# DiamondLightSource/fast-feedback-service

Hardware: AMD Instinct MI355X
Metric: detector frames/s (Eiger-16M 4362x4148 uint16) (higher is better)
Workload: dtype u16; 1 GPU; eiger16m: 4148x4362 uint16, 7x7 dispersion window, 32 frames/step/GPU resident in HBM, spots+centroids returned to host; streams=4, parallelism=single GPU, spot_gather=none (single GPU)

## Files before the change

fast-feedback-service_amd/csrc/ffs_context.hip:

```cpp
#include <sys/mman.h>

#include "ffs_internal.hpp"
#include "kernels_mask.hpp"

static_assert(sizeof(ReflOut) == sizeof(ffs_reflection), "record layout");
static_assert(offsetof(ReflOut, sum_intensity) == offsetof(ffs_reflection, sum_intensity), "record layout");

thread_local std::string g_create_error;

static void ctx_destroy_internal(ffs_ctx* c);
namespace {
struct Registry {
    std::mutex mu;
    std::unordered_set<const void*> live[3];
    std::atomic<bool> exiting{false};
    bool exit_hook_installed = false;
};
Registry& registry() {
    static Registry* r = new Registry();
    return *r;
}
static void on_process_exit() {
    Registry& r = registry();
    std::vector<ffs_ctx*> ctxs;
// ... 131 lines not shown
    }
    const uint64_t npx = (uint64_t)width * height;
    c->cap = max_strong ? max_strong : (uint32_t)std::min<uint64_t>(npx, 1u << 18);
    c->cap = (uint32_t)std::min<uint64_t>(c->cap, npx);
    c->max_comp = std::min<uint32_t>(c->cap, 1u << 14);
    c->n_tiles = ((int)height + kTileRows - 1) / kTileRows;
    ffs_default_params(&c->params);
    if (hipSetDevice(device) != hipSuccess) {
        g_create_error = "hipSetDevice failed";
        delete c;
        return FFS_ERR_DEVICE;
    }
    hipError_t e = hipMalloc(&c->d_maskbits, L.plane_frame_stride + 256);
    if (e == hipSuccess) e = hipMalloc(&c->d_ginfo, (size_t)(L.H + kInfoExtraRows) * ginfo_pitch(L, pixel_bytes) + 256);
    if (e == hipSuccess) e = hipMalloc(&c->d_mmap, (size_t)L.H * L.pitch_px + 256);
    if (e != hipSuccess) {
        g_create_error = std::string("hipMalloc(mask): ") + hipGetErrorString(e);
        ctx_destroy_internal(c);
        return FFS_ERR_NOMEM;
    }
    c->chain_ok = chain_prepare_device();
    {
        int lo = 0, hi = 0;
        hipError_t es = hipDeviceGetStreamPriorityRange(&lo, &hi);
        if (es == hipSuccess) es = hipStreamCreateWithPriority(&c->dense_st, hipStreamNonBlocking, (lo + hi) / 2);
        if (es == hipSuccess) es = hipStreamCreateWithFlags(&c->up_st, hipStreamNonBlocking);
        for (auto& sp : c->sparse_st)
            if (es == hipSuccess) es = hipStreamCreateWithPriority(&sp, hipStreamNonBlocking, hi);
        if (es == hipSuccess)
            for (auto& e : c->chain_ev)
// ... 97 lines not shown

static void ctx_destroy_internal(ffs_ctx* c) {
    (void)hipSetDevice(c->device);
    ahead_stop(c, true);
    for (auto* st : c->stack_pool) stack3d_free(st);
    c->stack_pool.clear();
    if (AssemblyPool* pool = c->assembly.exchange(nullptr)) {
        pool->owner.lock();
        pool->owner.unlock();
        delete pool;
    }
    if (c->d_maskbits) (void)hipFree(c->d_maskbits);
    if (c->d_gain_map) (void)hipFree(c->d_gain_map);
    if (c->d_ginfo) (void)hipFree(c->d_ginfo);
    if (c->d_mmap) (void)hipFree(c->d_mmap);
    if (c->dense_st) (void)hipStreamDestroy(c->dense_st);
    if (c->dense_st2) (void)hipStreamDestroy(c->dense_st2);
    if (c->d_handoff) (void)hipFree(c->d_handoff);
    if (c->up_st) (void)hipStreamDestroy(c->up_st);
    for (auto st : c->sparse_st) if (st) (void)hipStreamDestroy(st);
    for (auto e : c->chain_ev) if (e) (void)hipEventDestroy(e);
    for (auto& pb : c->pinned_pool) pinned_free(pb);
    delete c;
}

static int rebuild_mask_tables(ffs_ctx* c) {
    const Layout& L = c->L;
    const uint32_t gpitch = ginfo_pitch(L, c->pixel_bytes);
    HIP_TRY(c, hipMemset(c->d_ginfo, 0, (size_t)(L.H + kInfoExtraRows) * gpitch));
    const int groups = L.pitch_px / (c->pixel_bytes == 2 ? 8 : 4);
    (void)hipGetLastError();
    if (c->pixel_bytes == 2)
        hipLaunchKernelGGL(k_build_maps, dim3((groups + 255) / 256, L.H), dim3(256), 0, 0, c->d_maskbits, L.mpitch, L.W, L.H,
                           L.pitch_px, c->d_mmap, c->d_ginfo, gpitch);
    else
        hipLaunchKernelGGL(k_build_maps4, dim3((groups + 255) / 256, L.H), dim3(256), 0, 0, c->d_maskbits, L.mpitch, L.W, L.H,
                           L.pitch_px, c->d_mmap, c->d_ginfo, gpitch);
    HIP_TRY(c, hipGetLastError());
    HIP_TRY(c, hipDeviceSynchronize());
    return FFS_OK;
}

static int ffs_ctx_set_mask_impl(ffs_ctx* c, const uint8_t* host_mask) {
    if (!c) return FFS_ERR_INVALID;
    const Layout& L = c->L;
    std::vector<uint8_t> bits(L.plane_frame_stride, 0);
    const int full = L.W / 8;
    for (int y = 0; y < L.H; ++y) {
        uint8_t* row = bits.data() + (size_t)y * L.mpitch;
        if (host_mask) {
            const uint8_t* m = host_mask + (size_t)y * L.W;
            for (int g = 0; g < full; ++g) {
                uint64_t v;
                std::memcpy(&v, m + 8 * g, 8);
// ... 209 lines not shown
    else if (k == "sched") { if ((ok = (value == 0 || value == 3) && c->n_streams_made == 0)) t.sched = (int)value; }
    else if (k == "chain_first") { if ((ok = in(0, 64))) t.chain_first = (int)value; }
    else if (k == "bright_cap") { if ((ok = in(0, kBrightCap))) t.bright_cap = (int)value; }
    else if (k == "frames_per_group") { if ((ok = in(1, 1 << 30))) t.frames_per_group = (int)value; }
    else if (k == "target_waves") { if ((ok = in(1, 1 << 24))) t.target_waves = value; }
    else if (k == "stream_bands") { if ((ok = in(0, 4096))) t.stream_bands = (int)value; }
    else if (k == "dense_mask") { if ((ok = in(0, 1))) t.dense_mask = (int)value; }
    else if (k == "occupancy_bitmap") { if ((ok = in(0, 1))) t.occupancy_bitmap = (int)value; }
    else if (k == "direct_records") { if ((ok = in(0, 1) && c->n_streams_made == 0)) t.direct_records = (int)value; }
    else if (k == "decode_in_dense_stream") { if ((ok = in(0, 1))) t.decode_in_dense_stream = (int)value; }
    else if (k == "ext_fused") { if ((ok = in(0, 1))) t.ext_fused = (int)value; }
    else if (k == "ext_erode") { if ((ok = in(0, 2))) t.ext_erode = (int)value; }
    else if (k == "ext_e_sparse") { if ((ok = in(0, 1))) t.ext_e_sparse = (int)value; }
    else if (k == "ext_rest_aside") { if ((ok = in(0, 1))) t.ext_rest_aside = (int)value; }
    else if (k == "band_taper") { if ((ok = in(0, 99))) t.band_taper = (int)value; }
    else if (k == "rows_ahead") { if ((ok = in(2, 4))) t.rows_ahead = (int)value; }
    else if (k == "ccl_grid") { if ((ok = in(1, 1024))) t.ccl_grid = (int)value; }
    else {
        c->err = "ffs_ctx_set_tuning: unknown key '" + k + "'";
        return FFS_ERR_INVALID;
    }
    if (!ok) {
        c->err = "ffs_ctx_set_tuning: value out of range for '" + k + "' (sched / direct_records: before the first stream is created)";
        return FFS_ERR_INVALID;
    }
    return FFS_OK;
}


extern "C" void ffs_stream_destroy(ffs_stream* s) {
// ... 260 lines not shown
```

fast-feedback-service_amd/csrc/ffs_device.h:

```cpp
#pragma once
#include <hip/hip_runtime.h>
#include <stdint.h>

#include "launch_geometry.hpp"
#include "threshold_route.hpp"

#ifdef FFS_EXPERIMENTS
#define FFS_DBG(args, bit) (((args).dbg & (bit)) != 0)
#define FFS_STOP_AFTER(A, phase) if ((A).stop_after == (phase)) return
#define FFS_PHASE_TS(A, idx) do { if ((A).phase_ts && threadIdx.x == 0) (A).phase_ts[(size_t)blockIdx.x * 8 + (idx)] = wall_clock64(); } while (0)
#else
#define FFS_PHASE_TS(A, idx) do {} while (0)
#define FFS_DBG(args, bit) false
#define FFS_STOP_AFTER(A, phase) do {} while (0)
#endif

namespace ffsamd {

constexpr int kInfoExtraRows = 3;

constexpr int kWlogCap = 256;
constexpr int kTileRows = 8;
constexpr int kExactListCap = 2048;

// ... 21 lines not shown
    uint32_t ib2, is2;
    uint32_t thr_floor;
    int bright_to_plane;
    uint8_t* dplane;
    uint8_t* eplane;
    int eplane_clean;
    int ext_strips, ext_band_rows, ext_bands;
    int ext_flavour;
    int ext_variant;
    const uint8_t* ginfo;
    const uint8_t* mmap;
    uint32_t gpitch;
    int gpf;
    int n_frames;
    int group_frames;
    int s_strips, s_band_rows, s_bands;
    uint32_t* bright_n;
    uint2* bright_list;
    uint32_t bright_cap;
    uint32_t* overflow;
    uint32_t* occ;
    uint32_t occ_frame_words;
    uint32_t occ_spr;
    int dense_mask;
    uint2* wlog;
    uint32_t* wlog_n;
    uint4* wpix;
    uint32_t* handoff;
    uint32_t handoff_seq;
    int dbg_prio;
    int dbg;
// ... 157 lines not shown
```

fast-feedback-service_amd/csrc/ffs_internal.hpp:

```cpp
#pragma once
#include <algorithm>
#include <atomic>
#include <chrono>
#include <condition_variable>
#include <functional>
#include <cmath>
#include <cstdio>
#include <cstdlib>
#include <cstring>
#include <deque>
#include <map>
#include <mutex>
#include <new>
#include <string>
#include <thread>
#include <unordered_set>
#include <vector>

#include <hip/hip_runtime.h>
#include <hip/hip_ext.h>

#include "ffs_hip.h"
#include "ffs_device.h"
#include "threshold_route.hpp"
// ... 64 lines not shown
    Layout L{};
    int pixel_bytes = 2;
    uint32_t max_batch = 1;
    uint32_t cap = 0;
    uint32_t max_comp = 0;
    int n_tiles = 0;
    ffs_params params{};
    int max_valid_scope = FFS_MAX_VALID_CENTRE;
    double gain = 0.0;
    float* d_gain_map = nullptr;
    bool has_gain_map = false;
    float gain_map_min = 0.0f, gain_map_max = 0.0f;
    uint8_t* d_maskbits = nullptr;
    uint8_t* d_ginfo = nullptr;
    uint8_t* d_mmap = nullptr;
    hipStream_t dense_st = nullptr;
    hipStream_t dense_st2 = nullptr;
    uint32_t* d_handoff = nullptr;
    std::mutex dense_mu;
    uint32_t handoff_seq = 0;
    int handoff_last = -1;
    hipStream_t up_st = nullptr;
    hipStream_t sparse_st[2] = {nullptr, nullptr};
    int n_streams_made = 0;
    std::mutex stream_mu;
    std::vector<ffs_stream*> live_streams;
    std::vector<ffs_stack3d*> live_stacks;
    std::vector<ffs_stack3d*> stack_pool;
    std::vector<struct PinnedBuf> pinned_pool;
    std::atomic<int> inflight{0};
// ... 19 lines not shown
    ffs_stream* big = nullptr;
    std::vector<OverflowFrame> ovf;
    bool lists_valid = true;
    bool log_off = false;
    uint2* d_wlog = nullptr;
    uint32_t* d_wlog_n = nullptr;
    uint4* d_wpix = nullptr;
    size_t wlog_waves = 0;
    uint4* d_band_hdr = nullptr;
    uint8_t* d_band_acc = nullptr;
    uint32_t* d_band_seam = nullptr;
    uint32_t band_slots = 0;
    uint32_t band_backoff = 0;
    uint32_t path_bits = 0;
    uint32_t reruns = 0;
    bool runs_overflowed = false;
    uint32_t *d_pack_k = nullptr, *d_pack_i = nullptr;
    StackSlice *d_pack_tab = nullptr, *h_pack_tab = nullptr;
    hipEvent_t ev_pack = nullptr;
    hipEvent_t ev_sent = nullptr;
    int ev_sent_dev = -1;
    bool sent_pending = false;
    hipStream_t st = nullptr;
    hipStream_t st_up = nullptr;
    bool st2_shared = false;
    bool st_shared = false;
    hipStream_t st2 = nullptr;
    hipEvent_t ev[7] = {};
    uint8_t* d_slab = nullptr;
    uint8_t* d_img = nullptr;
// ... 174 lines not shown
```

fast-feedback-service_amd/csrc/ffs_submit.hip:

```cpp
#include "ffs_internal.hpp"
#include "kernels_threshold.hpp"
#include "kernels_extended.hpp"
#include "kernels_stream.hpp"
#include "kernels_ccl.hpp"
#include "kernels_chain.hpp"
#include "kernels_band.hpp"
#include "kernels_decode.hpp"
#include "kernels_byteoffset.hpp"
#include "kernels_window.hpp"

bool chain_prepare_device() {
    const hipError_t e1 = hipFuncSetAttribute(reinterpret_cast<const void*>(&k_frame_chain<uint16_t>), hipFuncAttributeMaxDynamicSharedMemorySize, kChainDynBytes);
    const hipError_t e2 = hipFuncSetAttribute(reinterpret_cast<const void*>(&k_frame_chain<uint32_t>), hipFuncAttributeMaxDynamicSharedMemorySize, kChainDynBytes);
    const hipError_t e3 = hipFuncSetAttribute(reinterpret_cast<const void*>(&k_frame_chain<uint16_t, true>), hipFuncAttributeMaxDynamicSharedMemorySize, kChainDynBytes);
    const hipError_t e4 = hipFuncSetAttribute(reinterpret_cast<const void*>(&k_frame_chain<uint16_t, false, true>), hipFuncAttributeMaxDynamicSharedMemorySize, kChainDynBytes);
    const hipError_t e5 = hipFuncSetAttribute(reinterpret_cast<const void*>(&k_frame_chain<uint32_t, false, true>), hipFuncAttributeMaxDynamicSharedMemorySize, kChainDynBytes);
    (void)hipGetLastError();
    return e1 == hipSuccess && e2 == hipSuccess && e3 == hipSuccess && e4 == hipSuccess && e5 == hipSuccess;
}

ThresholdRoute batch_route(const ffs_stream* s, const Rerun& how) {
    const ParamSnapshot& b = s->batch;
    return threshold_route(b.params.algorithm, s->ctx->pixel_bytes, win_default(b.params), b.max_valid_scope, b.params.max_valid, b.gain, how.threshold_path,
                           s->ctx->tune, b.gain_map);
// ... 20 lines not shown
    a.bright_to_plane = route.bright_to_plane;
    a.overflow = s->d_overflow;
    a.bright_n = s->d_tile_counts + tile_counts_bytes(s) / 4 - 1;
    a.bright_list = s->d_bright;
    a.bright_cap = std::min<uint32_t>(kBrightCap, (uint32_t)c->tune.bright_cap);
    a.occ = s->d_occ;
    a.occ_frame_words = occ_frame_words(L);
    a.occ_spr = L.mpitch / 16;
    a.dense_mask = (p.want_strong_mask || c->tune.dense_mask || a.bright_to_plane) ? 1 : 0;
#ifdef FFS_EXPERIMENTS
    a.dbg = c->tune.exp.k1_debug;
    if (a.dbg & 16) a.dense_mask = 1;
    if (a.dbg & 8) a.dense_mask = 0;
#endif
    a.dbg_prio = c->tune.stream_prio;
    a.ginfo = c->d_ginfo;
    a.mmap = c->d_mmap;
    a.gpitch = ginfo_pitch(L, c->pixel_bytes);
    a.gpf = groups_per_row(L, c->pixel_bytes);
    a.dplane = s->d_dplane;
    a.eplane = s->d_eplane;
    a.eplane_clean = s->ext_e_clean ? 1 : 0;
    a.ext_variant = route.ext_variant;
}
static void set_predicate(ThresholdArgs& a, const ffs_params& p, bool trusted, double gain, const ffs_ctx* map_of) {
    a.nb_limit = trusted ? (uint32_t)std::min<long long>(p.max_valid, (1ll << 24) - 1) + 1u : 1u << 24;
    a.kS = (float)(p.nsig_s * p.nsig_s * (1.0 - 1.0 / 65536.0));
    a.kB = (float)(p.nsig_b * (1.0 - 1.0 / 1048576.0));
    a.min_count = p.min_count;
    a.nsig_b = p.nsig_b;
// ... 65 lines not shown
}

static dim3 stream_grid(const ThresholdArgs& a, const StreamGeometry& g) {
    return dim3(8u * stream_chunk(a), (unsigned)g.n_groups);
}

using StreamKernel = void (*)(ThresholdArgs);
static StreamKernel stream_kernel(const ffs_ctx* c, bool dense_mask, bool extended) {
    const int rows = std::clamp(c->tune.rows_ahead, 2, c->pixel_bytes == 4 ? 3 : 4);
    if (c->pixel_bytes == 4) return dense_mask ? k_stream_u32<2, true> : rows == 3 ? k_stream_u32<3, false> : k_stream_u32<2, false>;
    if (extended) return dense_mask ? k_stream_u16<2, true, true> : k_stream_u16<2, true, false>;
    if (dense_mask) return k_stream_u16<2, false, true>;
    return rows == 4 ? k_stream_u16<4, false, false> : rows == 3 ? k_stream_u16<3, false, false> : k_stream_u16<2, false, false>;
}
static void launch_stream(ffs_stream* s, const ThresholdArgs& a, const StreamGeometry& g, hipEvent_t start, hipEvent_t stop, hipStream_t st = nullptr) {
    hipExtLaunchKernelGGL(stream_kernel(s->ctx, a.dense_mask != 0, false), stream_grid(a, g), dim3(64), 0, st ? st : s->st, start, stop, 0, a);
}
template <typename PixelT, Predicate V>
struct KernelTag {
    using pixel = PixelT;
    static constexpr Predicate of(KernelFamily f) { return instantiated_as(f, sizeof(PixelT), V); }
};
template <Predicate V, typename Launch>
static void with_pixel_tag(int pixel_bytes, Launch& launch) {
    if (pixel_bytes == 4) launch(KernelTag<uint32_t, V>{});
    else launch(KernelTag<uint16_t, V>{});
}
template <typename Launch>
static void with_kernel_tag(int pixel_bytes, Predicate v, Launch&& launch) {
    if (v == Predicate::kGainMap) with_pixel_tag<Predicate::kGainMap>(pixel_bytes, launch);
// ... 28 lines not shown
}
static void launch_exact(ffs_stream* s, const ThresholdRoute& route, const ThresholdArgs& a, uint32_t n_frames, hipStream_t st) {
    const dim3 grid((unsigned)a.n_tiles, n_frames);
    with_kernel_tag(s->ctx->pixel_bytes, route.variant, [&](auto tag) {
        using T = decltype(tag);
        if (route.window_3x3) hipLaunchKernelGGL((k_exact<typename T::pixel, T::of(KernelFamily::kExact)>), grid, dim3(256), 0, st, a);
        else hipLaunchKernelGGL((k_exact_w<typename T::pixel, T::of(KernelFamily::kExact)>), grid, dim3(256), 0, st, a);
    });
}

static void launch_ext_first(ffs_stream* s, const ThresholdRoute& route, const ThresholdArgs& a, const StreamGeometry& g, uint32_t n_frames, hipEvent_t start, hipEvent_t stop, bool fix_here = true,
                             bool plane_clean = false, bool counts_clean = false) {
    if (route.ext_streams_first()) {
        if (!plane_clean) (void)hipMemsetAsync(a.dplane, 0, (size_t)n_frames * a.plane_frame_stride, s->st);
        if (!counts_clean) (void)hipMemsetAsync(a.tile_counts, 0, tile_counts_bytes(s), s->st);
        hipExtLaunchKernelGGL(stream_kernel(s->ctx, a.dense_mask != 0, true), stream_grid(a, g), dim3(64), 0, s->st, start, stop, 0, a);
        if (fix_here) hipLaunchKernelGGL((k_bright_fix<uint16_t, true>), dim3(32), dim3(256), 0, s->st, a);
        return;
    }
    dim3 g1((unsigned)(a.ext_strips * a.ext_bands), n_frames);
    with_kernel_tag(s->ctx->pixel_bytes, route.variant, [&](auto tag) {
        using T = decltype(tag);
        hipExtLaunchKernelGGL((k_ext_first<typename T::pixel, T::of(KernelFamily::kExtFirst)>), g1, dim3(64), 0, s->st, start, stop, 0, a);
    });
}
static void launch_ext_rest(ffs_stream* s, const ThresholdRoute& route, const ThresholdArgs& a, uint32_t n_frames, hipStream_t st) {
    if (!route.ext_streams_first()) (void)hipMemsetAsync(a.strong_bytes, 0, (size_t)n_frames * a.bytes_frame_stride, st);
    dim3 g3((unsigned)a.n_tiles, n_frames);
    if (route.ext_fused) {
        hipLaunchKernelGGL(route.variant == Predicate::kWindowScope ? k_ext_erode_final<Predicate::kWindowScope> : k_ext_erode_final<Predicate::kPhotonCount>, g3,
// ... 521 lines not shown
        HIP_TRY(c, hipMemcpyAsync(s->h_recs, s->d_recs, s->spec_recs_copied * sizeof(WireRec2), hipMemcpyDeviceToHost, s->st2));
    }
    HIP_TRY(c, hipEventRecord(s->ev[4], s->st2));
    return finish_enqueue(s, n, plan.ext || skip_sparse, skip_sparse);
}

static int launch_sparse_stage(ffs_stream* s, const BatchPlan& plan) {
    const CclArgs ca = make_ccl_args(s, plan);
    const SegArgs sa = make_seg_args(s, plan);
    s->bits_cleared = ca.clear_bits != 0;
    s->lists_valid = !(plan.use_log || plan.runs_launch) || plan.need_lists;
    s->dense_valid = plan.want_dense_bytes;
    s->occ_dirty = !(ca.use_occ && plan.will_chain);
    s->chain_mode = plan.will_chain;
    s->path_bits = plan.path_bits;
    return plan.will_chain ? launch_one_launch_stage(s, plan, ca, sa) : launch_grid_stage(s, plan, ca, sa);
}

int enqueue_batch(ffs_stream* s, const void* d_img, size_t pitch, size_t fstride, uint32_t n, const ParamSnapshot* snapshot, const Rerun& how) {
    s->batch = snapshot ? *snapshot : snapshot_of(s->ctx);
    s->cur_img = d_img;
    s->cur_pitch = pitch;
    s->cur_fstride = fstride;
    (void)hipGetLastError();
    bool ext_plane_clean = false;
    FFS_TRY(take_extended_planes(s, ext_plane_clean));
    const BatchPlan plan = plan_batch(s, d_img, pitch, fstride, n, how);
    if (plan.use_log && s->band_backoff > 0 && !how.no_bands) --s->band_backoff;
    bool dense_resets = false;
    FFS_TRY(reset_for_batch(s, plan, dense_resets));
// ... 450 lines not shown
```

fast-feedback-service_amd/csrc/ffs_wait.hip:

```cpp
#include "ffs_internal.hpp"

static int ensure_list_host(ffs_stream* s) {
    ffs_ctx* c = s->ctx;
    if (!s->h_list_k) {
        const size_t bytes = (size_t)s->max_batch * s->cap * 4;
        HIP_TRY(c, hipHostMalloc(reinterpret_cast<void**>(&s->h_list_k), bytes, hipHostMallocDefault));
        HIP_TRY(c, hipHostMalloc(reinterpret_cast<void**>(&s->h_list_i), bytes, hipHostMallocDefault));
    }
    return FFS_OK;
}

static void place_frames(const ffs_stream* s, const std::vector<OverflowFrame>* ovf, std::vector<size_t>& box_at, std::vector<size_t>& refl_at,
                         std::vector<size_t>& rec_at) {
    const uint32_t n = s->n_frames;
    const size_t B = s->max_batch;
    const uint32_t* h_nc = s->h_counts + counts_comp_at(B);
    const uint32_t* h_sm = s->h_counts + counts_summary_at(B);
    const bool want_refl = s->batch.params.want_reflections != 0;
    size_t nb = 0, nr = 0, at = 0;
    for (uint32_t f = 0; f < n; ++f) {
        box_at[f] = nb;
        refl_at[f] = nr;
        const uint32_t nc = std::min<uint32_t>(h_nc[f], s->max_comp);
        rec_at[f] = s->chain_mode ? (size_t)f * s->max_comp : at;
// ... 495 lines not shown
    if (!s) return FFS_ERR_INVALID;
    if (boxes) *boxes = s->boxes.data();
    if (n_boxes) *n_boxes = (uint32_t)s->boxes.size();
    if (refls) *refls = s->refls.data();
    if (n_refls) *n_refls = (uint32_t)s->refls.size();
    return FFS_OK;
}

extern "C" int ffs_stream_last_path(ffs_stream* s, uint32_t* path_bits, uint32_t* reruns) {
    if (!s) return FFS_ERR_INVALID;
    if (path_bits) *path_bits = s->path_bits;
    if (reruns) *reruns = s->reruns;
    return FFS_OK;
}

extern "C" int ffs_stream_timings(ffs_stream* s, float ms[5]) {
    if (!s || !ms) return FFS_ERR_INVALID;
    if (s->timings_stale && !s->busy) {
        (void)hipSetDevice(s->ctx->device);
        s->timings[0] = 0.0f;
        if (!s->dev_input) (void)hipEventElapsedTime(&s->timings[0], s->ev[0], s->ev[1]);
        (void)hipEventElapsedTime(&s->timings[1], s->ev[1], s->ev[2]);
        (void)hipEventElapsedTime(&s->timings[2], s->ev[2], s->ev3_is_ev4 ? s->ev[4] : s->ev[3]);
        (void)hipEventElapsedTime(&s->timings[3], s->ev3_is_ev4 ? s->ev[4] : s->ev[3], s->timing_last);
        (void)hipEventElapsedTime(&s->timings[4], s->dev_input ? s->ev[1] : s->ev[0], s->timing_last);
        (void)hipGetLastError();
        s->timings_stale = false;
    }
    std::memcpy(ms, s->timings, sizeof(s->timings));
    return FFS_OK;
// ... 67 lines not shown
```

fast-feedback-service_amd/csrc/kernels_mask.hpp:

```cpp
#pragma once
#include "ffs_device.h"

namespace ffsamd {

__global__ __launch_bounds__(256) void k_build_maps(const uint8_t* maskbits, uint32_t mpitch, int W, int H, int pitch_px,
                                                    uint8_t* mmap, uint8_t* ginfo, uint32_t gpitch_bytes) {
    const int g = blockIdx.x * 256 + threadIdx.x;
    const int y = blockIdx.y;
    if (g * 8 >= pitch_px) return;
    uint32_t cnt[8] = {0, 0, 0, 0, 0, 0, 0, 0};
    for (int dy = -3; dy <= 3; ++dy) {
        const int yy = y + dy;
        if (yy < 0 || yy >= H) continue;
        const uint8_t* row = maskbits + (uint64_t)yy * mpitch;
        uint32_t b = (uint32_t)row[g] << 8;
        if (g > 0) b |= row[g - 1];
        if ((uint32_t)(g + 1) < mpitch) b |= (uint32_t)row[g + 1] << 16;
        for (int j = 0; j < 8; ++j) cnt[j] += __popc((b >> (j + 5)) & 0x7Fu);
    }
    const uint32_t own = maskbits[(uint64_t)y * mpitch + g];
    uint32_t mn = 255, mx = 0;
    for (int j = 0; j < 8; ++j) {
        mmap[(uint64_t)y * pitch_px + g * 8 + j] = (uint8_t)cnt[j];
        if ((own >> j) & 1u) { mn = min(mn, cnt[j]); mx = max(mx, cnt[j]); }
// ... 22 lines not shown
        for (int j = 0; j < 4; ++j) cnt[j] += __popc((b >> (5 + sh + j)) & 0x7Fu);
    }
    const uint32_t own = (maskbits[(uint64_t)y * mpitch + byte0] >> sh) & 0xFu;
    uint32_t mn = 255, mx = 0;
    for (int j = 0; j < 4; ++j) {
        mmap[(uint64_t)y * pitch_px + g * 4 + j] = (uint8_t)cnt[j];
        if ((own >> j) & 1u) { mn = min(mn, cnt[j]); mx = max(mx, cnt[j]); }
    }
    if (mx == 0) mn = 0;
    ginfo[(uint64_t)y * gpitch_bytes + g * 4] = (uint8_t)own;
    ginfo[(uint64_t)(y + kInfoExtraRows) * gpitch_bytes + g * 4 + 1] = (uint8_t)mn;
    ginfo[(uint64_t)(y + kInfoExtraRows) * gpitch_bytes + g * 4 + 2] = (uint8_t)mx;
    ginfo[(uint64_t)(y + kInfoExtraRows) * gpitch_bytes + g * 4 + 3] = (uint8_t)own;
}


__global__ void k_resolution_mask(uint8_t* maskbits, uint32_t mpitch, int W, int H, float wavelength,
                                  float distance, float cx, float cy, float psx, float psy,
                                  float dmin, float dmax) {
    const int bx = blockIdx.x * blockDim.x + threadIdx.x;
    const int y = blockIdx.y;
    if (bx * 8 >= W || y >= H) return;
    uint8_t* p = maskbits + (uint64_t)y * mpitch + bx;
    uint32_t b = *p;
    for (int j = 0; j < 8; ++j) {
        const int x = bx * 8 + j;
        if (x >= W || !((b >> j) & 1u)) continue;
        const float dx = (((float)x + 0.5f) - cx) * psx;
        const float dy = (((float)y + 0.5f) - cy) * psy;
        const float r = sqrtf(dx * dx + dy * dy);
// ... 9 lines not shown
```

fast-feedback-service_amd/csrc/kernels_stream.hpp:

```cpp
#pragma once
#include "kernels_threshold.hpp"

#ifndef FFS_IMG_LOAD_AUX
#define FFS_IMG_LOAD_AUX 0
#endif

namespace ffsamd {

constexpr int kSQWords = 32;

__device__ __forceinline__ bool exact_predicate(const ThresholdArgs& a, uint32_t m, unsigned long long sx,
                                                unsigned long long sy, uint32_t pc) {
    const double src = (double)pc;
    if (!((int)m >= a.min_count && src > a.threshold)) return false;
    if (a.max_valid >= 0 && (long long)pc > a.max_valid) return false;
    const double md = (double)m, xd = (double)sx, yd = (double)sy;
    const double t0 = md * yd;
    const double t1 = xd * xd;
    const double t2 = xd * (md - 1.0);
    const double av = (t0 - t1) - t2;
    const double bv = md * src - xd;
    const double cv = (xd * a.nsig_b) * __builtin_sqrt(2.0 * (md - 1.0));
    const double dv = a.nsig_s * __builtin_sqrt(xd * md);
    return av > cv && bv > dv;
// ... 71 lines not shown
__global__ __launch_bounds__(64, 4) void k_stream_u16(const ThresholdArgs a) {
    __shared__ uint32_t s_q[kSQWords][kQCap];
    __shared__ uint16_t s_list[kQCap * 8];

    const int lane = threadIdx.x;
    if (a.dbg_prio & 1) __builtin_amdgcn_s_setprio(3);
    int strip, band;
    const bool real = stream_unit(a, blockIdx.x, strip, band);
    if constexpr (!EXT)
        if (a.handoff && blockIdx.x == gridDim.x - 1 && blockIdx.y == gridDim.y - 1 && lane == 0)
            __hip_atomic_store(a.handoff, a.handoff_seq, __ATOMIC_RELEASE, __HIP_MEMORY_SCOPE_SYSTEM);
    if (!real) return;
    [[maybe_unused]] const uint32_t slot = log_slot(a, blockIdx.y, (uint32_t)band, (uint32_t)strip);
    const int f0 = blockIdx.y * a.group_frames;
    const int nf = min(a.group_frames, a.n_frames - f0);
    const int yb0 = band_first_row(band, a.band_rows, a.band_rows2, a.band_split);
    const int yb1 = min(band_first_row(band + 1, a.band_rows, a.band_rows2, a.band_split), a.H);

    const int gsep = a.gpf + 1;
    const int G = strip * kSOwned + lane - 1;
    const int fl = G >= 0 ? G / gsep : 0;
    const int g = G - fl * gsep;
    const bool active = G >= 0 && fl < nf && g < a.gpf;
    const bool owned = active && lane >= 1 && lane <= kSOwned;
    const uint32_t my_fg = ((uint32_t)fl << 16) | (uint32_t)g;

    const rsrc_t r_img = make_rsrc((const uint8_t*)a.image + (uint64_t)f0 * a.frame_stride,
                                   (uint32_t)((uint64_t)(nf - 1) * a.frame_stride + (uint64_t)a.H * a.pitch));
    const rsrc_t r_info = make_rsrc(a.ginfo, (uint32_t)(a.H + kInfoExtraRows) * a.gpitch);
    const rsrc_t r_sb = make_rsrc(a.strong_bytes + (uint64_t)f0 * a.bytes_frame_stride,
                                  (uint32_t)((uint64_t)nf * a.bytes_frame_stride));
    const rsrc_t r_cb = make_rsrc((EXT ? a.dplane : a.bits) + (uint64_t)f0 * a.plane_frame_stride, (uint32_t)((uint64_t)nf * a.plane_frame_stride));
// ... 404 lines not shown

template <int KAHEAD, bool DENSE = false>
__global__ __launch_bounds__(64, 4) void k_stream_u32(const ThresholdArgs a) {
    __shared__ uint32_t s_q[kS4Words][kQCap];
    __shared__ uint16_t s_list[kQCap * 4];

    const int lane = threadIdx.x;
    int strip, band;
    const bool real = stream_unit(a, blockIdx.x, strip, band);
    if (a.handoff && blockIdx.x == gridDim.x - 1 && blockIdx.y == gridDim.y - 1 && lane == 0)
        __hip_atomic_store(a.handoff, a.handoff_seq, __ATOMIC_RELEASE, __HIP_MEMORY_SCOPE_SYSTEM);
    if (!real) return;
    const uint32_t slot = log_slot(a, blockIdx.y, (uint32_t)band, (uint32_t)strip);
    const int f0 = blockIdx.y * a.group_frames;
    const int nf = min(a.group_frames, a.n_frames - f0);
    const int yb0 = band_first_row(band, a.band_rows, a.band_rows2, a.band_split);
    const int yb1 = min(band_first_row(band + 1, a.band_rows, a.band_rows2, a.band_split), a.H);

    const int gsep = a.gpf + 1;
    const int G = strip * kSOwned + lane - 1;
    const int fl = G >= 0 ? G / gsep : 0;
    const int g = G - fl * gsep;
    const bool active = G >= 0 && fl < nf && g < a.gpf;
    const bool owned = active && lane >= 1 && lane <= kSOwned;

    const rsrc_t r_img = make_rsrc((const uint8_t*)a.image + (uint64_t)f0 * a.frame_stride,
                                   (uint32_t)((uint64_t)(nf - 1) * a.frame_stride + (uint64_t)a.H * a.pitch));
    const rsrc_t r_info = make_rsrc(a.ginfo, (uint32_t)(a.H + kInfoExtraRows) * a.gpitch);
    const rsrc_t r_sb = make_rsrc(a.strong_bytes + (uint64_t)f0 * a.bytes_frame_stride,
                                  (uint32_t)((uint64_t)nf * a.bytes_frame_stride));
    constexpr uint32_t kOob = 0x80000000u;
    const uint32_t off_px = active ? (uint32_t)((uint64_t)fl * a.frame_stride) + (uint32_t)g * 16u : kOob;
// ... 295 lines not shown
```

fast-feedback-service_amd/csrc/launch_geometry.hpp:

```cpp
#pragma once
#include <stddef.h>
#include <stdint.h>

#include <algorithm>
#include <cmath>

#include "tuning.hpp"

#if defined(__HIPCC__)
#define FFS_HD __host__ __device__
#else
#define FFS_HD
#endif

namespace ffsamd {

struct Layout {
    int W, H;
    int pitch_px;
    uint32_t pitch;
    uint32_t mpitch;
    uint32_t bpitch;
    uint64_t frame_stride;
    uint64_t plane_frame_stride;
// ... 113 lines not shown
    ExtGeometry a{};
    a.ext_strips = (L.pitch_px + kExtOwnedPx - 1) / kExtOwnedPx;
    {
        const long long ext_target = 8192;
        long long er = ((long long)L.H * a.ext_strips * n_frames + 4 * ext_target - 1) / (4 * ext_target);
        er = std::max<long long>(64, std::min<long long>(er, 256));
        a.ext_band_rows = (int)er;
        a.ext_bands = (L.H + a.ext_band_rows - 1) / a.ext_band_rows;
    }
    return a;
}

FFS_HD inline int band_first_row(int band, int band_rows, int band_rows2, int band_split) {
    return band < band_split ? band * band_rows : band_split * band_rows + (band - band_split) * band_rows2;
}
FFS_HD inline uint32_t stream_units_of(int n_bands, int n_strips) { return (uint32_t)n_bands * (uint32_t)n_strips; }
FFS_HD inline uint32_t stream_chunk_of(int n_bands, int n_strips) { return (stream_units_of(n_bands, n_strips) + 7u) / 8u; }
FFS_HD inline bool stream_unit_of(uint32_t bid, int n_bands, int n_strips, int& strip, int& band) {
    const uint32_t u = (bid & 7u) * stream_chunk_of(n_bands, n_strips) + (bid >> 3);
    band = (int)(u / (uint32_t)n_strips);
    strip = (int)(u - (uint32_t)band * (uint32_t)n_strips);
    return u < stream_units_of(n_bands, n_strips);
}
FFS_HD inline uint32_t log_slot_of(int n_bands, int n_strips, uint32_t y, uint32_t band, uint32_t strip) {
    return (y * (uint32_t)n_bands + band) * (uint32_t)n_strips + strip;
}

}
```

fast-feedback-service_amd/csrc/tuning.hpp:

```cpp
#pragma once

namespace ffsamd {

struct Tuning {
    int threshold_path = 0;
    int ext_first_pass = 2;
    int sparse_stage = 2;
    int sched = 3;
    int chain_first = 2;
    int bright_cap = 1 << 20;
    int frames_per_group = 1 << 30;
    long long target_waves = 16384;
    int stream_bands = 0;
    int dense_mask = 0;
    int occupancy_bitmap = 1;
    int direct_records = 1;
    int decode_in_dense_stream = 1;
    int ccl_grid = 32;
    int ext_erode = 2;
    int ext_e_sparse = 0;
    int ext_fused = 0;
    int ext_rest_aside = 0;
    int band_taper = 0;
    int rows_ahead = 3;
    int device_lists = 2;
    int strong_log = 1;
    int chain_runs = 1;
    int sparse_bands = 1;
    int dense_overlap = 0;
    int stream_prio = 1;
    int assembly_threads = 7;
    int wait_ahead = 1;
    int sparse_priority = 0;
    int window_kernel = 0;
#ifdef FFS_EXPERIMENTS
    struct Exp {
        int k1_debug = 0, chain_skip = 0, chain_stop = 0, dummy_us = 0, dummy_wg = 32, dummy_threads = 1024, dummy_lds = 0;
    } exp;
// ... 5 lines not shown
```

fast-feedback-service_amd/python/ffs_amd/api.py:

```python
from __future__ import annotations

import ctypes as C
import os
from dataclasses import dataclass, field

import numpy as np

_PKG = os.path.dirname(os.path.dirname(os.path.dirname(os.path.abspath(__file__))))


def lib_path() -> str:
    return os.environ.get("FFS_HIP_LIB") or os.path.join(_PKG, "libffs_hip.so")


class FfsError(RuntimeError):
    def __init__(self, code: int, msg: str):
        super().__init__(f"libffs_hip error {code}: {msg}")
        self.code = code


class Params(C.Structure):
    _fields_ = [("min_count", C.c_int32), ("nsig_b", C.c_double), ("nsig_s", C.c_double),
                ("threshold", C.c_double), ("max_valid", C.c_int64),
                ("min_spot_size", C.c_uint32), ("min_spot_size_3d", C.c_uint32),
# ... 46 lines not shown

MAX_VALID_CENTRE, MAX_VALID_WINDOW = 0, 1

CODEC_BSLZ4 = 0
CODEC_BYTE_OFFSET = 1

EXPORTS = [
    "ffs_default_params", "ffs_device_count", "ffs_device_name", "ffs_device_total_mem",
    "ffs_ctx_create", "ffs_ctx_destroy", "ffs_last_error", "ffs_ctx_set_mask",
    "ffs_ctx_apply_resolution_mask", "ffs_ctx_get_mask", "ffs_ctx_set_params",
    "ffs_stream_create", "ffs_stream_destroy", "ffs_stream_host_buffer", "ffs_submit",
    "ffs_submit_device", "ffs_ctx_device_layout", "ffs_wait", "ffs_stream_batch_arrays", "ffs_stream_timings",
    "ffs_submit_compressed", "ffs_decode_only", "ffs_submit_encoded", "ffs_decode_only_encoded", "ffs_stream_spot_centres", "ffs_bench_threshold", "ffs_bench_hbm", "ffs_stream_debug_planes", "ffs_stream_debug_bitplane", "ffs_selftest_sqrt", "ffs_stack3d_create",
    "ffs_stack3d_destroy", "ffs_stack3d_add_batch", "ffs_stack3d_add_slice", "ffs_stack3d_finish", "ffs_stack3d_signals", "ffs_stack3d_last_finish_ms", "ffs_multi_init", "ffs_multi_transport",
    "ffs_ctx_set_tuning", "ffs_bench_pipeline", "ffs_device_numa_node", "ffs_stream_reserve_host", "ffs_stream_last_path", "ffs_multi_gather_rows",
    "ffs_ctx_set_max_valid_scope", "ffs_ctx_set_gain", "ffs_ctx_set_gain_map",
]

_lib = None


def load_library():
    global _lib
    if _lib is None:
        p = lib_path()
        if not os.path.exists(p):
            raise RuntimeError(f"{p} is missing: run `make hip` or __graft_entry__.build(). "
                               "There is no CPU fallback for the product path.")
        L = C.CDLL(p)
        L.ffs_last_error.restype = C.c_char_p
        L.ffs_last_error.argtypes = [C.c_void_p]
# ... 326 lines not shown
        self.submit(frames, first_frame_id)
        return self.wait()

    def timings(self):
        t = (C.c_float * 5)()
        self.ctx._check(self._lib.ffs_stream_timings(self._h, t))
        return dict(zip(("h2d", "threshold", "ccl", "d2h", "total"), list(t)))

    PATH_BITS = {"wave_logs": 1, "frame_chain": 2, "bands": 4, "runs": 8, "grid_kernels": 16, "extended": 32, "window": 64}

    def last_path(self):
        bits, reruns = C.c_uint32(), C.c_uint32()
        self.ctx._check(self._lib.ffs_stream_last_path(self._h, C.byref(bits), C.byref(reruns)))
        return {k for k, v in self.PATH_BITS.items() if bits.value & v}, reruns.value

    def bench_threshold(self, dev_ptr: int, pitch_bytes: int, frame_stride_bytes: int, n_frames: int,
                        iters: int):
        a, b = C.c_float(), C.c_float()
        self.ctx._check(self._lib.ffs_bench_threshold(self._h, C.c_void_p(dev_ptr), pitch_bytes,
                                                      frame_stride_bytes, n_frames, iters,
                                                      C.byref(a), C.byref(b)))
        return a.value, b.value

    def bench_hbm(self, iters: int = 5):
        a, b = C.c_float(), C.c_float()
        self.ctx._check(self._lib.ffs_bench_hbm(self._h, iters, C.byref(a), C.byref(b)))
        return a.value, b.value

    def pack_spot_centres(self, out: np.ndarray, cap: int) -> int:
        assert out.dtype == np.float32 and out.flags.c_contiguous and out.size >= (cap + 1) * 4
# ... 107 lines not shown
```

include/ffs_hip.h:

```cpp
#ifndef FFS_HIP_H
#define FFS_HIP_H

#include <stddef.h>
#include <stdint.h>

#ifdef __cplusplus
extern "C" {
#endif

#pragma GCC visibility push(default)

#define FFS_OK 0
#define FFS_ERR_INVALID (-1)
#define FFS_ERR_DEVICE (-2)
#define FFS_ERR_NOMEM (-3)
#define FFS_ERR_OVERFLOW (-4)
#define FFS_ERR_NODEVICE (-5)

typedef struct ffs_ctx ffs_ctx;
typedef struct ffs_stream ffs_stream;
typedef struct ffs_stack3d ffs_stack3d;

typedef struct {
    int32_t min_count;
// ... 111 lines not shown

int ffs_stream_batch_arrays(ffs_stream *s, const ffs_box **boxes, uint32_t *n_boxes,
                            const ffs_reflection **reflections, uint32_t *n_reflections);

int ffs_stream_timings(ffs_stream *s, float ms[5]);

#define FFS_PATH_WAVE_LOGS 1u
#define FFS_PATH_FRAME_CHAIN 2u
#define FFS_PATH_BANDS 4u
#define FFS_PATH_RUNS 8u
#define FFS_PATH_GRID_KERNELS 16u
#define FFS_PATH_EXTENDED 32u
#define FFS_PATH_WINDOW 64u
int ffs_stream_last_path(ffs_stream *s, uint32_t *path_bits, uint32_t *reruns);

int ffs_stream_spot_centres(ffs_stream *s, float *rows4, uint32_t cap, uint32_t *n_written);

int ffs_bench_threshold(ffs_stream *s, const void *device_pixels, size_t pitch_bytes,
                        size_t frame_stride_bytes, uint32_t n_frames, uint32_t iters,
                        float *ms_dense, float *ms_rest);
int ffs_bench_pipeline(ffs_stream *const *streams, uint32_t n_streams, const void *device_pixels,
                       size_t pitch_bytes, size_t frame_stride_bytes, uint32_t n_frames, uint32_t steps,
                       int64_t first_frame_id, uint64_t *n_boxes, uint64_t *n_strong_pixels);
int ffs_bench_hbm(ffs_stream *s, uint32_t iters, float *read_gbps, float *mix_gbps);
int ffs_stream_debug_planes(ffs_stream *s, const uint8_t **device_strong_bytes,
                            size_t *mask_pitch, size_t *mask_frame_stride);
int ffs_stream_debug_bitplane(ffs_stream *s, uint32_t frame_in_batch, int which, uint8_t *host_out);

int ffs_selftest_sqrt(ffs_ctx *ctx, uint64_t begin, uint64_t end, uint64_t *sum_of_bits);

// ... 24 lines not shown
```

Measured before the change: 112,500 frames/s.

## Trim streaming kernel bands to rows with valid mask pixels

Builds a per-row bitmap recording which detector rows contain any unmasked pixel, and the streaming threshold kernels shrink each band's row range to the first and last live rows, exiting early when a band has none. This avoids reading and processing fully masked rows such as module gaps. It adds a small bitmap build at mask time, a host copy used for diagnostics, and a new query API. It also removes unused strip/band fields from the argument struct.

```diff
diff --git a/fast-feedback-service_amd/csrc/ffs_context.hip b/fast-feedback-service_amd/csrc/ffs_context.hip
--- a/fast-feedback-service_amd/csrc/ffs_context.hip
+++ b/fast-feedback-service_amd/csrc/ffs_context.hip
@@ -169,6 +169,7 @@
     hipError_t e = hipMalloc(&c->d_maskbits, L.plane_frame_stride + 256);
     if (e == hipSuccess) e = hipMalloc(&c->d_ginfo, (size_t)(L.H + kInfoExtraRows) * ginfo_pitch(L, pixel_bytes) + 256);
     if (e == hipSuccess) e = hipMalloc(&c->d_mmap, (size_t)L.H * L.pitch_px + 256);
+    if (e == hipSuccess) e = hipMalloc(reinterpret_cast<void**>(&c->d_rowbits), row_bitmap_words(L.H) * 4);
     if (e != hipSuccess) {
         g_create_error = std::string("hipMalloc(mask): ") + hipGetErrorString(e);
         ctx_destroy_internal(c);
@@ -296,6 +297,7 @@
     if (c->d_gain_map) (void)hipFree(c->d_gain_map);
     if (c->d_ginfo) (void)hipFree(c->d_ginfo);
     if (c->d_mmap) (void)hipFree(c->d_mmap);
+    if (c->d_rowbits) (void)hipFree(c->d_rowbits);
     if (c->dense_st) (void)hipStreamDestroy(c->dense_st);
     if (c->dense_st2) (void)hipStreamDestroy(c->dense_st2);
     if (c->d_handoff) (void)hipFree(c->d_handoff);
@@ -318,8 +320,11 @@
     else
         hipLaunchKernelGGL(k_build_maps4, dim3((groups + 255) / 256, L.H), dim3(256), 0, 0, c->d_maskbits, L.mpitch, L.W, L.H,
                            L.pitch_px, c->d_mmap, c->d_ginfo, gpitch);
+    hipLaunchKernelGGL(k_build_rowbits, dim3((unsigned)row_bitmap_words(L.H)), dim3(64), 0, 0, c->d_maskbits, L.mpitch, L.H, c->d_rowbits);
     HIP_TRY(c, hipGetLastError());
     HIP_TRY(c, hipDeviceSynchronize());
+    c->h_rowbits.resize(row_bitmap_words(L.H));
+    HIP_TRY(c, hipMemcpy(c->h_rowbits.data(), c->d_rowbits, c->h_rowbits.size() * 4, hipMemcpyDeviceToHost));
     return FFS_OK;
 }
 
@@ -559,6 +564,7 @@
     else if (k == "ext_e_sparse") { if ((ok = in(0, 1))) t.ext_e_sparse = (int)value; }
     else if (k == "ext_rest_aside") { if ((ok = in(0, 1))) t.ext_rest_aside = (int)value; }
     else if (k == "band_taper") { if ((ok = in(0, 99))) t.band_taper = (int)value; }
+    else if (k == "trim_rows") { if ((ok = in(0, 1))) t.trim_rows = (int)value; }
     else if (k == "rows_ahead") { if ((ok = in(2, 4))) t.rows_ahead = (int)value; }
     else if (k == "ccl_grid") { if ((ok = in(1, 1024))) t.ccl_grid = (int)value; }
     else {
diff --git a/fast-feedback-service_amd/csrc/ffs_device.h b/fast-feedback-service_amd/csrc/ffs_device.h
--- a/fast-feedback-service_amd/csrc/ffs_device.h
+++ b/fast-feedback-service_amd/csrc/ffs_device.h
@@ -59,7 +59,7 @@
     int gpf;
     int n_frames;
     int group_frames;
-    int s_strips, s_band_rows, s_bands;
+    const uint32_t* rowbits;
     uint32_t* bright_n;
     uint2* bright_list;
     uint32_t bright_cap;
diff --git a/fast-feedback-service_amd/csrc/ffs_internal.hpp b/fast-feedback-service_amd/csrc/ffs_internal.hpp
--- a/fast-feedback-service_amd/csrc/ffs_internal.hpp
+++ b/fast-feedback-service_amd/csrc/ffs_internal.hpp
@@ -102,6 +102,8 @@
     uint8_t* d_maskbits = nullptr;
     uint8_t* d_ginfo = nullptr;
     uint8_t* d_mmap = nullptr;
+    uint32_t* d_rowbits = nullptr;
+    std::vector<uint32_t> h_rowbits;
     hipStream_t dense_st = nullptr;
     hipStream_t dense_st2 = nullptr;
     uint32_t* d_handoff = nullptr;
@@ -151,6 +153,8 @@
     uint32_t band_backoff = 0;
     uint32_t path_bits = 0;
     uint32_t reruns = 0;
+    bool trim_on = false;
+    StreamGeometry trim_geo{};
     bool runs_overflowed = false;
     uint32_t *d_pack_k = nullptr, *d_pack_i = nullptr;
     StackSlice *d_pack_tab = nullptr, *h_pack_tab = nullptr;
diff --git a/fast-feedback-service_amd/csrc/ffs_submit.hip b/fast-feedback-service_amd/csrc/ffs_submit.hip
--- a/fast-feedback-service_amd/csrc/ffs_submit.hip
+++ b/fast-feedback-service_amd/csrc/ffs_submit.hip
@@ -58,6 +58,7 @@
     if (a.dbg & 8) a.dense_mask = 0;
 #endif
     a.dbg_prio = c->tune.stream_prio;
+    a.rowbits = (c->tune.trim_rows && !a.dense_mask) ? c->d_rowbits : nullptr;
     a.ginfo = c->d_ginfo;
     a.mmap = c->d_mmap;
     a.gpitch = ginfo_pitch(L, c->pixel_bytes);
@@ -153,6 +154,8 @@
     return rows == 4 ? k_stream_u16<4, false, false> : rows == 3 ? k_stream_u16<3, false, false> : k_stream_u16<2, false, false>;
 }
 static void launch_stream(ffs_stream* s, const ThresholdArgs& a, const StreamGeometry& g, hipEvent_t start, hipEvent_t stop, hipStream_t st = nullptr) {
+    s->trim_on = a.rowbits != nullptr;
+    s->trim_geo = g;
     hipExtLaunchKernelGGL(stream_kernel(s->ctx, a.dense_mask != 0, false), stream_grid(a, g), dim3(64), 0, st ? st : s->st, start, stop, 0, a);
 }
 template <typename PixelT, Predicate V>
@@ -211,6 +214,8 @@
     if (route.ext_streams_first()) {
         if (!plane_clean) (void)hipMemsetAsync(a.dplane, 0, (size_t)n_frames * a.plane_frame_stride, s->st);
         if (!counts_clean) (void)hipMemsetAsync(a.tile_counts, 0, tile_counts_bytes(s), s->st);
+        s->trim_on = a.rowbits != nullptr;
+        s->trim_geo = g;
         hipExtLaunchKernelGGL(stream_kernel(s->ctx, a.dense_mask != 0, true), stream_grid(a, g), dim3(64), 0, s->st, start, stop, 0, a);
         if (fix_here) hipLaunchKernelGGL((k_bright_fix<uint16_t, true>), dim3(32), dim3(256), 0, s->st, a);
         return;
@@ -762,6 +767,7 @@
     s->occ_dirty = !(ca.use_occ && plan.will_chain);
     s->chain_mode = plan.will_chain;
     s->path_bits = plan.path_bits;
+    if (plan.window || plan.route.stage == ThresholdStage::kCrossCheck || (plan.ext && !plan.route.ext_streams_first())) s->trim_geo = StreamGeometry{};
     return plan.will_chain ? launch_one_launch_stage(s, plan, ca, sa) : launch_grid_stage(s, plan, ca, sa);
 }
 
diff --git a/fast-feedback-service_amd/csrc/ffs_wait.hip b/fast-feedback-service_amd/csrc/ffs_wait.hip
--- a/fast-feedback-service_amd/csrc/ffs_wait.hip
+++ b/fast-feedback-service_amd/csrc/ffs_wait.hip
@@ -533,6 +533,17 @@
     return FFS_OK;
 }
 
+extern "C" int ffs_stream_last_trim(ffs_stream* s, int* trimmed, uint64_t* rows_planned, uint64_t* rows_run) {
+    if (!s) return FFS_ERR_INVALID;
+    const ffs_ctx* c = s->ctx;
+    const bool launched = s->trim_geo.n_bands > 0, on = launched && s->trim_on && c->h_rowbits.size() == row_bitmap_words(c->L.H);
+    const RowIterations r = launched ? stream_row_iterations(s->trim_geo, c->L.H, on ? c->h_rowbits.data() : nullptr) : RowIterations{0, 0};
+    if (trimmed) *trimmed = on ? 1 : 0;
+    if (rows_planned) *rows_planned = r.planned;
+    if (rows_run) *rows_run = r.trimmed;
+    return FFS_OK;
+}
+
 extern "C" int ffs_stream_timings(ffs_stream* s, float ms[5]) {
     if (!s || !ms) return FFS_ERR_INVALID;
     if (s->timings_stale && !s->busy) {
diff --git a/fast-feedback-service_amd/csrc/kernels_mask.hpp b/fast-feedback-service_amd/csrc/kernels_mask.hpp
--- a/fast-feedback-service_amd/csrc/kernels_mask.hpp
+++ b/fast-feedback-service_amd/csrc/kernels_mask.hpp
@@ -60,6 +60,18 @@
     ginfo[(uint64_t)(y + kInfoExtraRows) * gpitch_bytes + g * 4 + 3] = (uint8_t)own;
 }
 
+__global__ __launch_bounds__(64) void k_build_rowbits(const uint8_t* maskbits, uint32_t mpitch, int H, uint32_t* rowbits) {
+    const int lane = threadIdx.x;
+    uint32_t word = 0;
+    for (int r = 0; r < 32; ++r) {
+        const int y = (int)blockIdx.x * 32 + r;
+        if (y >= H) break;
+        uint32_t any = 0;
+        for (uint32_t b = (uint32_t)lane; b < mpitch; b += 64u) any |= maskbits[(uint64_t)y * mpitch + b];
+        if (__ballot(any != 0u) != 0ull) word |= 1u << r;
+    }
+    if (lane == 0) rowbits[blockIdx.x] = word;
+}
 
 __global__ void k_resolution_mask(uint8_t* maskbits, uint32_t mpitch, int W, int H, float wavelength,
                                   float distance, float cx, float cy, float psx, float psy,
diff --git a/fast-feedback-service_amd/csrc/kernels_stream.hpp b/fast-feedback-service_amd/csrc/kernels_stream.hpp
--- a/fast-feedback-service_amd/csrc/kernels_stream.hpp
+++ b/fast-feedback-service_amd/csrc/kernels_stream.hpp
@@ -109,8 +109,17 @@
     [[maybe_unused]] const uint32_t slot = log_slot(a, blockIdx.y, (uint32_t)band, (uint32_t)strip);
     const int f0 = blockIdx.y * a.group_frames;
     const int nf = min(a.group_frames, a.n_frames - f0);
-    const int yb0 = band_first_row(band, a.band_rows, a.band_rows2, a.band_split);
-    const int yb1 = min(band_first_row(band + 1, a.band_rows, a.band_rows2, a.band_split), a.H);
+    RowRange rows = {band_first_row(band, a.band_rows, a.band_rows2, a.band_split), min(band_first_row(band + 1, a.band_rows, a.band_rows2, a.band_split), a.H)};
+    if constexpr (!DENSE) {
+        if (a.rowbits && rows.y1 > rows.y0) {
+            rows = trim_band_rows((const __attribute__((address_space(4))) uint32_t*)a.rowbits, rows.y0, rows.y1);
+            if (rows.y1 == rows.y0) {
+                if constexpr (!EXT) if (a.wlog && lane == 0) a.wlog_n[slot] = 0u;
+                return;
+            }
+        }
+    }
+    const int yb0 = rows.y0, yb1 = rows.y1;
 
     const int gsep = a.gpf + 1;
     const int G = strip * kSOwned + lane - 1;
@@ -545,8 +554,17 @@
     const uint32_t slot = log_slot(a, blockIdx.y, (uint32_t)band, (uint32_t)strip);
     const int f0 = blockIdx.y * a.group_frames;
     const int nf = min(a.group_frames, a.n_frames - f0);
-    const int yb0 = band_first_row(band, a.band_rows, a.band_rows2, a.band_split);
-    const int yb1 = min(band_first_row(band + 1, a.band_rows, a.band_rows2, a.band_split), a.H);
+    RowRange rows = {band_first_row(band, a.band_rows, a.band_rows2, a.band_split), min(band_first_row(band + 1, a.band_rows, a.band_rows2, a.band_split), a.H)};
+    if constexpr (!DENSE) {
+        if (a.rowbits && rows.y1 > rows.y0) {
+            rows = trim_band_rows((const __attribute__((address_space(4))) uint32_t*)a.rowbits, rows.y0, rows.y1);
+            if (rows.y1 == rows.y0) {
+                if (a.wlog && lane == 0) a.wlog_n[slot] = 0u;
+                return;
+            }
+        }
+    }
+    const int yb0 = rows.y0, yb1 = rows.y1;
 
     const int gsep = a.gpf + 1;
     const int G = strip * kSOwned + lane - 1;
diff --git a/fast-feedback-service_amd/csrc/launch_geometry.hpp b/fast-feedback-service_amd/csrc/launch_geometry.hpp
--- a/fast-feedback-service_amd/csrc/launch_geometry.hpp
+++ b/fast-feedback-service_amd/csrc/launch_geometry.hpp
@@ -151,6 +151,45 @@
 FFS_HD inline int band_first_row(int band, int band_rows, int band_rows2, int band_split) {
     return band < band_split ? band * band_rows : band_split * band_rows + (band - band_split) * band_rows2;
 }
+inline size_t row_bitmap_words(int H) { return ((size_t)H + 31) / 32; }
+struct RowRange { int y0, y1; };
+template <typename Words>
+FFS_HD inline RowRange trim_band_rows(Words bits, int yb0, int yb1) {
+    const int w0 = yb0 >> 5, w1 = (yb1 - 1) >> 5;
+    uint32_t lo = bits[w0] & (0xFFFFFFFFu << (yb0 & 31));
+    uint32_t hi = bits[w1] & (0xFFFFFFFFu >> (31 - ((yb1 - 1) & 31)));
+    if (w0 == w1) lo = hi = lo & hi;
+    int w = w0;
+    uint32_t v = lo;
+    while (v == 0u && w < w1) {
+        ++w;
+        v = w == w1 ? hi : bits[w];
+    }
+    if (v == 0u) return {yb0, yb0};
+    const int y0 = w * 32 + __builtin_ctz(v);
+    w = w1;
+    v = hi;
+    while (v == 0u) {
+        --w;
+        v = w == w0 ? lo : bits[w];
+    }
+    return {y0, w * 32 + 32 - __builtin_clz(v)};
+}
+struct RowIterations { uint64_t planned, trimmed; };
+inline RowIterations stream_row_iterations(const StreamGeometry& g, int H, const uint32_t* bits) {
+    RowIterations r{0, 0};
+    for (int band = 0; band < g.n_bands; ++band) {
+        const int yb0 = band_first_row(band, g.band_rows, g.band_rows2, g.band_split);
+        const int yb1 = std::min(band_first_row(band + 1, g.band_rows, g.band_rows2, g.band_split), H);
+        if (yb1 <= yb0) continue;
+        r.planned += (uint64_t)(yb1 - yb0) + 6;
+        if (!bits) { r.trimmed += (uint64_t)(yb1 - yb0) + 6; continue; }
+        const RowRange t = trim_band_rows(bits, yb0, yb1);
+        if (t.y1 > t.y0) r.trimmed += (uint64_t)(t.y1 - t.y0) + 6;
+    }
+    return r;
+}
+
 FFS_HD inline uint32_t stream_units_of(int n_bands, int n_strips) { return (uint32_t)n_bands * (uint32_t)n_strips; }
 FFS_HD inline uint32_t stream_chunk_of(int n_bands, int n_strips) { return (stream_units_of(n_bands, n_strips) + 7u) / 8u; }
 FFS_HD inline bool stream_unit_of(uint32_t bid, int n_bands, int n_strips, int& strip, int& band) {
diff --git a/fast-feedback-service_amd/csrc/tuning.hpp b/fast-feedback-service_amd/csrc/tuning.hpp
--- a/fast-feedback-service_amd/csrc/tuning.hpp
+++ b/fast-feedback-service_amd/csrc/tuning.hpp
@@ -22,6 +22,7 @@
     int ext_fused = 0;
     int ext_rest_aside = 0;
     int band_taper = 0;
+    int trim_rows = 1;
     int rows_ahead = 3;
     int device_lists = 2;
     int strong_log = 1;
diff --git a/fast-feedback-service_amd/python/ffs_amd/api.py b/fast-feedback-service_amd/python/ffs_amd/api.py
--- a/fast-feedback-service_amd/python/ffs_amd/api.py
+++ b/fast-feedback-service_amd/python/ffs_amd/api.py
@@ -84,7 +84,7 @@
     "ffs_submit_compressed", "ffs_decode_only", "ffs_submit_encoded", "ffs_decode_only_encoded", "ffs_stream_spot_centres", "ffs_bench_threshold", "ffs_bench_hbm", "ffs_stream_debug_planes", "ffs_stream_debug_bitplane", "ffs_selftest_sqrt", "ffs_stack3d_create",
     "ffs_stack3d_destroy", "ffs_stack3d_add_batch", "ffs_stack3d_add_slice", "ffs_stack3d_finish", "ffs_stack3d_signals", "ffs_stack3d_last_finish_ms", "ffs_multi_init", "ffs_multi_transport",
     "ffs_ctx_set_tuning", "ffs_bench_pipeline", "ffs_device_numa_node", "ffs_stream_reserve_host", "ffs_stream_last_path", "ffs_multi_gather_rows",
-    "ffs_ctx_set_max_valid_scope", "ffs_ctx_set_gain", "ffs_ctx_set_gain_map",
+    "ffs_ctx_set_max_valid_scope", "ffs_ctx_set_gain", "ffs_ctx_set_gain_map", "ffs_stream_last_trim",
 ]
 
 _lib = None
@@ -441,6 +441,13 @@
         self.ctx._check(self._lib.ffs_stream_last_path(self._h, C.byref(bits), C.byref(reruns)))
         return {k for k, v in self.PATH_BITS.items() if bits.value & v}, reruns.value
 
+    def last_trim(self):
+        fn = self._lib.ffs_stream_last_trim
+        fn.argtypes = [C.c_void_p, C.POINTER(C.c_int), C.POINTER(C.c_uint64), C.POINTER(C.c_uint64)]
+        on, planned, run = C.c_int(), C.c_uint64(), C.c_uint64()
+        self.ctx._check(fn(self._h, C.byref(on), C.byref(planned), C.byref(run)))
+        return bool(on.value), planned.value, run.value
+
     def bench_threshold(self, dev_ptr: int, pitch_bytes: int, frame_stride_bytes: int, n_frames: int,
                         iters: int):
         a, b = C.c_float(), C.c_float()
diff --git a/include/ffs_hip.h b/include/ffs_hip.h
--- a/include/ffs_hip.h
+++ b/include/ffs_hip.h
@@ -149,6 +149,8 @@
 #define FFS_PATH_WINDOW 64u
 int ffs_stream_last_path(ffs_stream *s, uint32_t *path_bits, uint32_t *reruns);
 
+int ffs_stream_last_trim(ffs_stream *s, int *trimmed, uint64_t *rows_planned, uint64_t *rows_run);
+
 int ffs_stream_spot_centres(ffs_stream *s, float *rows4, uint32_t cap, uint32_t *n_written);
 
 int ffs_bench_threshold(ffs_stream *s, const void *device_pixels, size_t pitch_bytes,
```

New measurement: 115,200 frames/s (median of 6 runs). 2.4% higher.
